# xXCoffeeColaXc/WeatherConverter

Measured on AMD Instinct MI355X. Metric: 256x256 images/sec (T=1000 DDPM sample), higher is better.
Workload: dtype fp32-class (f16x3: 2-piece fp16 split MFMA, fp32 accumulate); 1 GPU; DDPM reverse sampling, UNet config.yaml @ 256px, 16 images/GPU, T=1000, 127 timed steps from t=999; global_batch=16, image_size=256, parallelism=single GPU, devices=1, hip_graph=True, stream_groups=2, x_finite=True

## Files before the change

weatherconverter_amd/csrc/wc_wino.hip:

```cpp
#include <stdlib.h>

#include "wc_x6.hpp"

#ifndef WC_ABL
#define WC_ABL 0
#endif
#ifndef WC_WINO_SCALAR
#define WC_WINO_SCALAR 0
#endif

namespace {

using namespace wcx6;

constexpr int NT = 256;

WC_DEVICE void wino_lds16(__amdgpu_buffer_rsrc_t srd, void* dst, unsigned voff, int soff) {
    __builtin_amdgcn_raw_ptr_buffer_load_lds(srd, (__attribute__((address_space(3))) void*)dst, 16, voff, soff, 0, 0);
}

struct WDev {
    const float* src0;
    int C0, ldc0;
    const float* scale;
    const float* shift;
    const float* src1;
    int C1, ldc1;
    int B, H, W, N;
    const void* w;
    const float* bias;
    const float* temb;
    int temb_ld;
    const float* res;
    int ldres;
    float* out;
    int ldo;
    int nck0, nck1;
    int a_exp;
    const float* abound;
    const float* wsinv;
    float* absmax;
    float* gn_part;
    int gn_ncb, gn_sw, gn_c0, gn_np64;
    int tiles_x, tiles_y, ntiles_n;
    const unsigned char* vpre;
    long vimg;
    const float* gb_x;
    int gb_ldx, gb_silu;
    const float* gb_sc0;
    const float* gb_sh0;
    const float* gb_gamma;
    const float* gb_beta;
    float* gb_part;
    float* gb_part3;
};

WC_DEVICE float wino_silu_grad(float y) {
    const float s = 1.0f / (1.0f + __expf(-y));
    return s * (1.0f + y * (1.0f - s));
}

constexpr int VPL = WC_SINGLE16 ? 8 : 16;

template <int TH, int BN, int MB = 2, int NW = 4, bool VP = false>
struct WTile {
    static constexpr int NT = 64 * NW;
    static constexpr int WAVES_N = BN / 32;
    static constexpr int WAVES_M = NW / WAVES_N;
    static_assert(WAVES_N * WAVES_M == NW && WAVES_M * 4 * MB == TH, "each wave owns 4 MB rows x 8 tiles x 32 channels");
    static constexpr int PBN = BN > 128 ? 128 : BN;
    static constexpr int HR = TH + 2;
    static constexpr int PSTR = HR * 128 + (VP ? 0 : 16);
    static constexpr int DPIECES = VPL * HR * 8 / 64;
    static_assert(!VP || VPL * HR * 8 == DPIECES * 64, "VP: the halo stage is a whole number of 1-KiB pieces");
    static constexpr int DPW = (DPIECES + NW - 1) / NW;
    static constexpr int HSTAGE = 16 * PSTR;
    static constexpr int CPSTR = TH * 128 + 16;
    static constexpr int CSTAGE = 8 * CPSTR;
    static constexpr int ITEMS = HR * 16;
    static constexpr int I_PER_T = (ITEMS + NT - 1) / NT;
    static constexpr int C_PER_T = TH * 16 * 4 / NT;
    static constexpr int BSTEP = PBN * 64;
    static constexpr int STEPS = 12;
};

WC_DEVICE int wg_grp(int r) { return ((r >= 4 && r < 12) || (r >= 16 && r < 20) || r >= 28) ? 1 : 0; }
WC_DEVICE int wg_idx(int r) { return r < 4 ? r : r < 12 ? r - 4 : r < 20 ? r - 8 : r < 28 ? r - 12 : r - 16; }
WC_DEVICE int wg_row(int r) { return 2 * wg_grp(r) + (wg_idx(r) >> 3); }
WC_DEVICE int wg_tile(int r) { return wg_idx(r) & 7; }

template <int TH, int BN, int PRO, bool RES, int MB = 2, int NW = 4>
__global__ __launch_bounds__(64 * NW) __attribute__((amdgpu_waves_per_eu(MB == 4 ? 1 : 2, MB == 4 ? 1 : 2)))
void conv3x3_wino_kernel(WDev p) {
    static_assert((PRO == 2 || PRO == 0 || PRO == 3) && !(PRO == 0 && RES),
                  "GN+SiLU (+ residual), pre-split GN+SiLU (+ residual) or one raw segment");
    constexpr bool VP = PRO == 3;
    using T = WTile<TH, BN, MB, NW, VP>;
    constexpr int NT = T::NT;
    extern __shared__ __attribute__((aligned(16))) unsigned char smem[];
    unsigned char* const cbase = smem + 2 * T::HSTAGE;

    const int tid = threadIdx.x;
    const int lane = tid & 63;
    const int wave = tid >> 6;
    const int wm = wave / T::WAVES_N;
    const int wn = wave % T::WAVES_N;

    const int nblk = gridDim.x;
    int bid = blockIdx.x;
    {
        int q = nblk / 8, r = nblk % 8, xcd = bid % 8;
        bid = (xcd < r ? xcd * (q + 1) : r * (q + 1) + (xcd - r) * q) + bid / 8;
    }
    const int tile_n = bid % p.ntiles_n;
    int tt = bid / p.ntiles_n;
    const int txi = tt % p.tiles_x;
    tt /= p.tiles_x;
    const int tyi = tt % p.tiles_y;
    const int b = tt / p.tiles_y;
    const int y0 = tyi * TH, x0 = txi * 16, n0 = tile_n * BN;

    int s_exp = p.a_exp;
    if ((RES || PRO == 0) && p.abound) {
        const float bnd = p.abound[b];
        const int e = (int)((__float_as_uint(bnd) >> 23) & 0xffu) - 127;
        if (bnd > 0.f) s_exp = min(s_exp, (PRO == 0 ? 12 : 13) - e);
        s_exp = max(s_exp, -100);
    }
    const float ascale = ldexpf(1.0f, s_exp), ainv = ldexpf(1.0f, -s_exp);
    const int S0 = T::STEPS * p.nck0;
    const int S = S0 + (RES ? p.nck1 : 0);
    constexpr bool RI = RES && (T::C_PER_T <= 2 || MB == 4);
    const int nri = RI ? min(p.nck0, p.nck1) : 0;
    const int ntail = RES ? p.nck1 - nri : 0;
    constexpr int WPT = T::PBN / 32;
    const unsigned wtile = (unsigned)(tile_n * (BN / T::PBN) + wn / WPT) * (unsigned)(S * T::BSTEP);

    const __amdgpu_buffer_rsrc_t srd0 = make_srd(p.src0);
    const __amdgpu_buffer_rsrc_t srd1 = make_srd(RES ? p.src1 : p.src0);
    const __amdgpu_buffer_rsrc_t srdw = make_srd(p.w);
    const __amdgpu_buffer_rsrc_t srdsc = make_srd(PRO == 2 ? p.scale : p.src0);
    const __amdgpu_buffer_rsrc_t srdsh = make_srd(PRO == 2 ? p.shift : p.src0);
    const __amdgpu_buffer_rsrc_t srdv = make_srd(VP ? (const void*)(p.vpre + (long)b * p.vimg) : (const void*)p.src0);
    unsigned voff[VP ? T::DPW : 1];
    if constexpr (VP) {
#pragma unroll
        for (int i = 0; i < T::DPW; ++i) {
            const int f = (wave + NW * i) * 64 + lane;
            const int P = f / (T::HR * 8), r = (f >> 3) % T::HR, tl = f & 7;
            const int y = y0 - 1 + r;
            voff[i] = (unsigned)y < (unsigned)p.H ? (unsigned)(((P * p.H + y) * (p.W / 2) + (x0 >> 1) + tl) * 16) : OOB;
        }
    }
    const int vchunk = VPL * p.H * (p.W / 2) * 16;
    auto dma_halo = [&](int c, int hs) {
        if constexpr (VP) {
            unsigned char* dst = smem + hs * T::HSTAGE + wave * 1024;
#pragma unroll
            for (int i = 0; i < T::DPW; ++i)
                if (T::DPIECES % NW == 0 || wave + NW * i < T::DPIECES)
                    wino_lds16(srdv, dst + i * NW * 1024, voff[i], c * vchunk);
        }
    };

    const int q = tid & 3;
    int hbase[T::I_PER_T];
    unsigned hin[T::I_PER_T];
    int hwr[T::I_PER_T];
    const int hpx = p.ldc0 * 4;
#pragma unroll
    for (int j = 0; j < T::I_PER_T; ++j) {
        const int i = tid + NT * j;
        const int hrow = i >> 4, tp = (i >> 2) & 3;
        const bool valid = i < T::ITEMS;
        const int iy = y0 - 1 + hrow;
        hin[j] = 0;
#pragma unroll
        for (int k = 0; k < 6; ++k) {
            const int ix = x0 - 1 + 4 * tp + k;
            const bool inb = valid && (unsigned)iy < (unsigned)p.H && (unsigned)ix < (unsigned)p.W;
            hin[j] |= (inb ? 1u : 0u) << k;
        }
        hbase[j] = (((b * p.H + iy) * p.W + x0 - 1 + 4 * tp) * p.ldc0 + 4 * q) * 4;
        hwr[j] = valid ? (q >> 1) * T::PSTR + (hrow * 8 + 2 * tp) * 16 + (q & 1) * 8 : -1;
    }
    f32x4 rh[T::I_PER_T][6];
    f32x4 rsc, rsh;
    auto load_ss = [&](int c) {
        if constexpr (PRO == 2) {
            const unsigned o = (unsigned)(b * p.C0 + c * 16 + 4 * q) * 4u;
            rsc = bload_f4(srdsc, o);
            rsh = bload_f4(srdsh, o);
        }
    };
    auto load_slot = [&](int j, int c) {
#pragma unroll
        for (int k = 0; k < 6; ++k)
            rh[j][k] = bload_f4s(srd0, ((hin[j] >> k) & 1u) ? (unsigned)(hbase[j] + k * hpx) : OOB, c * 64);
    };
    auto load_halo = [&](int c) {
        if constexpr (VP) return;
#pragma unroll
        for (int j = 0; j < T::I_PER_T; ++j) load_slot(j, c);
        load_ss(c);
    };
#if WC_WINO_SCALAR
    const float cu = -1.4426950408889634f * ainv;
    auto prologue = [&](int j, int k0, int k1) {
        if constexpr (PRO == 2) {
            if (j == 0 && k0 == 0) {
                rsc = rsc * ascale;
                rsh = rsh * ascale;
            }
        }
        auto act = [&](f32x4 a) {
#pragma unroll
            for (int e = 0; e < 4; ++e) {
                float v;
                if constexpr (PRO == 2) {
                    const float ap = __builtin_fmaf(a[e], rsc[e], rsh[e]);
                    const float r = __builtin_amdgcn_rcpf(1.0f + __builtin_amdgcn_exp2f(ap * cu));
                    v = ap * r;
                } else {
                    v = a[e] * ascale;
                }
                a[e] = v;
            }
            return a;
        };
#pragma unroll
        for (int k = k0; k < k1; ++k) {
            const f32x4 zero = {0.f, 0.f, 0.f, 0.f};
#if WC_WINO_SCALAR == 2
            rh[j][k] = ((hin[j] >> k) & 1u) ? act(rh[j][k]) : zero;
#else
            const f32x4 a = act(rh[j][k]);
            rh[j][k] = ((hin[j] >> k) & 1u) ? a : zero;
#endif
        }
    };
#else
    auto prologue = [&](int j, int k0, int k1) {
#pragma unroll
        for (int k = k0; k < k1; ++k) {
            f32x4 a = rh[j][k];
            if constexpr (PRO == 2 && !(WC_ABL & 2)) {
                a = a * rsc + rsh;
                if constexpr (!(WC_ABL & 1)) {
                    a.x = silu_fast(a.x); a.y = silu_fast(a.y);
                    a.z = silu_fast(a.z); a.w = silu_fast(a.w);
                }
            }
            rh[j][k] = ((hin[j] >> k) & 1u) ? a * ascale : f32x4{0.f, 0.f, 0.f, 0.f};
        }
    };
#endif
    auto transform = [&](int j, int t, int hs, int p0 = 0, int p1 = 4) {
        if (hwr[j] < 0) return;
        unsigned char* base = smem + hs * T::HSTAGE + hwr[j] + t * 16;
        const f32x4 d0 = rh[j][2 * t], d1 = rh[j][2 * t + 1], d2 = rh[j][2 * t + 2], d3 = rh[j][2 * t + 3];
#if WC_WINO_SCALAR
        f32x4 V[4];
#pragma unroll
        for (int e = 0; e < 4; ++e) {
            V[0][e] = d0[e] - d2[e];
            V[1][e] = d1[e] + d2[e];
            V[2][e] = d2[e] - d1[e];
            V[3][e] = d1[e] - d3[e];
        }
#else
        const f32x4 V[4] = {d0 - d2, d1 + d2, d2 - d1, d1 - d3};
#endif
#pragma unroll
        for (int pos = p0; pos < p1; ++pos) {
            u32x2 a0, a1;
            split2_f16(V[pos], a0, a1);
            unsigned char* d = base + pos * 2 * T::PSTR;
            *reinterpret_cast<u32x2*>(d) = a0;
            *reinterpret_cast<u32x2*>(d + 8 * T::PSTR) = a1;
        }
    };
    auto write_items = [&](int hs) {
        if constexpr (VP) return;
#pragma unroll
        for (int j = 0; j < T::I_PER_T; ++j) {
            prologue(j, 0, 6);
            transform(j, 0, hs);
            transform(j, 1, hs);
        }
    };

    f32x4 rc[2][RES ? T::C_PER_T : 1];
    const int cpx = (tid >> 2) & 15, crow0 = tid >> 6;
    const unsigned coff0 = (unsigned)(((b * p.H + y0 + crow0) * p.W + x0 + cpx) * p.ldc1 + 4 * q);
    const unsigned cstep = (unsigned)(NW * p.W * p.ldc1);
    const int cwr0 = (cpx & 1) * 2 * T::CPSTR + (q >> 1) * T::CPSTR + (crow0 * 8 + (cpx >> 1)) * 16 + (q & 1) * 8;
    auto load_centre = [&](auto P, int c, bool live = true) {
        constexpr int PV = decltype(P)::value;
        const unsigned v = live ? coff0 * 4u : OOB;
#pragma unroll
        for (int j = 0; j < T::C_PER_T; ++j)
            rc[PV][j] = bload_f4s(srd1, v, (int)(((unsigned)j * cstep + (unsigned)c * 16u) * 4u));
    };
    auto write_centre = [&](auto P, int cs) {
        constexpr int PV = decltype(P)::value;
        unsigned char* base = cbase + cs * T::CSTAGE + cwr0;
        const float sg = (cpx & 1) ? -ascale : ascale;
#pragma unroll
        for (int j = 0; j < T::C_PER_T; ++j) {
            u32x2 a0, a1;
            split2_f16(rc[PV][j] * sg, a0, a1);
            unsigned char* d = base + j * NW * 8 * 16;
            *reinterpret_cast<u32x2*>(d) = a0;
            *reinterpret_cast<u32x2*>(d + 4 * T::CPSTR) = a1;
        }
    };

    const int l32 = lane & 31;
    const int half = lane >> 5;
    int abase[MB];
#pragma unroll
    for (int mb = 0; mb < MB; ++mb) abase[mb] = ((4 * MB * wm + 4 * mb + wg_row(l32)) * 8 + wg_tile(l32)) * 16;
    const unsigned wlane = (unsigned)(half * T::PBN * 16 + ((wn % WPT) * 32 + l32) * 16);

    u32x4 wreg[3][2];
    auto load_w = [&](int set, int st) {
        int s = st < S0 ? st : S0 + nri + (st - S0);
        s = s < S ? s : S - 1;
        const int off = (int)(wtile + (unsigned)s * T::BSTEP);
#pragma unroll
        for (int pc = 0; pc < 2; ++pc) wreg[set][pc] = bload_u4s(srdw, wlane + (unsigned)(pc * 2 * T::PBN * 16), off);
    };
    u32x4 wres[2];
    auto load_wres = [&](int r) {
        const int s = S0 + r < S ? S0 + r : S - 1;
        const int off = (int)(wtile + (unsigned)s * T::BSTEP);
#pragma unroll
        for (int pc = 0; pc < 2; ++pc) wres[pc] = bload_u4s(srdw, wlane + (unsigned)(pc * 2 * T::PBN * 16), off);
    };

    f32x16 acc[4][MB];
#pragma unroll
    for (int i = 0; i < 4; ++i)
#pragma unroll
        for (int j = 0; j < MB; ++j)
#pragma unroll
            for (int r = 0; r < 16; ++r) acc[i][j][r] = 0.f;

    u32x4 fa[2][MB][2];
    auto read_a = [&](int fs, int hs, int dy, int pos) {
        const unsigned char* ha = smem + hs * T::HSTAGE + (pos * 2 + half) * T::PSTR + dy * 128;
#pragma unroll
        for (int mb = 0; mb < MB; ++mb)
#pragma unroll
            for (int pc = 0; pc < 2; ++pc)
                fa[fs][mb][pc] = *reinterpret_cast<const u32x4*>(ha + pc * 8 * T::PSTR + abase[mb]);
    };
    auto mfma_a = [&](int fs, int set, int pos) {
#pragma unroll
        for (int mb = 0; mb < MB; ++mb) acc[pos][mb] = mfma_f16(fa[fs][mb][0], wreg[set][0], acc[pos][mb]);
#pragma unroll
        for (int mb = 0; mb < MB; ++mb) {
            acc[pos][mb] = mfma_f16c(fa[fs][mb][0], wreg[set][1], acc[pos][mb]);
            acc[pos][mb] = mfma_f16c(fa[fs][mb][1], wreg[set][0], acc[pos][mb]);
        }
    };
    auto compute_res = [&](const u32x4 (&w)[2], int cs) {
        const unsigned char* ca = cbase + cs * T::CSTAGE + half * T::CPSTR;
#pragma unroll
        for (int r = 0; r < 2; ++r) {
            u32x4 fr[MB][2];
#pragma unroll
            for (int mb = 0; mb < MB; ++mb)
#pragma unroll
                for (int pc = 0; pc < 2; ++pc)
                    fr[mb][pc] = *reinterpret_cast<const u32x4*>(ca + (pc * 4 + r * 2) * T::CPSTR + abase[mb]);
#pragma unroll
            for (int mb = 0; mb < MB; ++mb) {
                f32x16& a = acc[r ? 3 : 0][mb];
                a = mfma_f16(fr[mb][0], w[0], a);
                a = mfma_f16c(fr[mb][0], w[1], a);
                a = mfma_f16c(fr[mb][1], w[0], a);
            }
        }
    };

    const std::integral_constant<int, 0> I0;
    const std::integral_constant<int, 1> I1;
    const int pv0 = (p.nck0 - 1) & 1;
    load_halo(0);
    dma_halo(0, pv0);
    if constexpr (RI) load_centre(I0, 0, nri > 0);
    load_w(0, 0);
    load_w(1, 1);
    write_items(pv0);
    if constexpr (RI) write_centre(I0, pv0);
    if constexpr (VP) asm volatile("s_waitcnt vmcnt(0)" ::: "memory");
    __syncthreads();
    constexpr int HALO_AT = T::I_PER_T == 1 ? 2 : 3;
    auto load_at = [](int j) { return T::I_PER_T == 1 ? 2 : (j == 0 ? 3 : 7); };
    auto pro_at = [](int j) { return j == 0 ? 5 : 9; };
    auto slot_work = [&](int j, int k, int hs) {
        if constexpr (VP) return;
        if constexpr (WC_ABL & 4) {
            if (k >= 0 && k < 3) prologue(j, 2 * k, 2 * k + 2);
            return;
        }
        if constexpr (T::I_PER_T == 1) {
            if (k >= 0 && k < 3) prologue(j, 2 * k, 2 * k + 2);
            if (k >= 3 && k < 7) transform(j, (k - 3) >> 1, hs, ((k - 3) & 1) * 2, ((k - 3) & 1) * 2 + 2);
        } else {
            if (k == 0) prologue(j, 0, 6);
            if (k == 1 || k == 2) transform(j, k - 1, hs);
        }
    };
    auto chunk = [&](auto P, auto L, int c) {
        constexpr int PV = decltype(P)::value;
        constexpr bool LAST = decltype(L)::value != 0;
        read_a(0, PV, 0, 0);
#pragma unroll
        for (int st = 0; st < T::STEPS; ++st) {
            if (!(WC_ABL & 8) || c == 0) load_w((st + 2) % 3, T::STEPS * c + st + 2);
            if constexpr (!LAST) {
#pragma unroll
                for (int j = 0; j < T::I_PER_T; ++j)
                    if (!(WC_ABL & 32) && st == load_at(j)) load_slot(j, c + 1);
                if (st == HALO_AT) {
                    dma_halo(c + 1, PV ^ 1);
                    load_ss(c + 1);
                    if constexpr (RI) load_centre(I0, c + 1, c + 1 < nri);
                }
            } else if constexpr (RES) {
                if (st == HALO_AT) load_centre(I0, nri, ntail > 0);
                if (st == HALO_AT + 1) load_centre(I1, nri + 1, ntail > 1);
            }
            if constexpr (RI) {
                if (st == 9) load_wres(c);
            }
            __builtin_amdgcn_sched_barrier(0);
            if (st + 1 < T::STEPS && (!(WC_ABL & 64) || c == 0)) read_a((st + 1) & 1, PV, (st + 1) >> 2, (st + 1) & 3);
            mfma_a(st & 1, st % 3, st & 3);
            if constexpr (!LAST) {
#pragma unroll
                for (int j = 0; j < T::I_PER_T; ++j) slot_work(j, st - pro_at(j), PV ^ 1);
                if constexpr (RI) {
                    if (st == 9) write_centre(I0, PV ^ 1);
                }
            }
        }
        if constexpr (RES) {
            if constexpr (RI) {
                if (c < nri) compute_res(wres, PV);
            }
            if constexpr (LAST) {
                if (ntail > 0) write_centre(I0, 1);
            }
        }
        if constexpr (VP && !LAST) asm volatile("s_waitcnt vmcnt(4)" ::: "memory");
        if constexpr (!(WC_ABL & 16)) __syncthreads();
    };
    const std::integral_constant<int, 0> NL;
    const std::integral_constant<int, 1> LL;
    {
        int c = 0;
        if (pv0) chunk(I1, NL, c++);
        for (; c + 1 < p.nck0 - 1; c += 2) {
            chunk(I0, NL, c);
            chunk(I1, NL, c + 1);
        }
        chunk(I0, LL, p.nck0 - 1);
    }
    if constexpr (RES) {
        auto tstep = [&](auto P, int k) {
            constexpr int PV = decltype(P)::value;
            compute_res(wreg[PV], PV ^ 1);
            load_w(PV, S0 + k + 2);
            load_centre(P, nri + k + 2, k + 2 < ntail);
            __builtin_amdgcn_sched_barrier(0);
            if (k + 1 < ntail) write_centre(std::integral_constant<int, PV ^ 1>{}, PV);
            __syncthreads();
        };
        int k = 0;
        for (; k + 1 < ntail; k += 2) {
            tstep(I0, k);
            tstep(I1, k + 1);
        }
        if (k < ntail) tstep(I0, k);
    }

    const long img_px = (long)b * p.H * p.W;
    const __amdgpu_buffer_rsrc_t srd_out = make_srd(p.out + img_px * p.ldo);
    const __amdgpu_buffer_rsrc_t srd_res = make_srd(p.res ? p.res + img_px * p.ldres : p.out);
    const int n = n0 + wn * 32 + l32;
    const bool nok = n < p.N;
    float eadd = (nok && p.bias) ? p.bias[n] : 0.f;
    if (nok && p.temb) eadd += p.temb[b * p.temb_ld + n];
    const float emul = nok ? p.wsinv[n] * ainv : 0.f;
    float vmax = 0.f;
    float gs1 = 0.f, gs2 = 0.f, gs3 = 0.f;
    const int so_px = 4 * p.ldo;
    const int so_rs = 4 * p.ldres;
#pragma unroll
    for (int mb = 0; mb < MB; ++mb) {
        unsigned vo[4], vr[4];
#pragma unroll
        for (int j = 0; j < 4; ++j) {
            const int row = 8 * j + 4 * half;
            const int pix = (y0 + 4 * MB * wm + 4 * mb + wg_row(row)) * p.W + x0 + 2 * wg_tile(row);
            vo[j] = (unsigned)(pix * p.ldo + n) * 4u;
            vr[j] = (unsigned)(pix * p.ldres + (nok ? n : 0)) * 4u;
        }
        float rv[2][16];
        if (p.res) {
#pragma unroll
            for (int r = 0; r < 16; ++r) {
                rv[0][r] = bload_f1s(srd_res, vr[r >> 2], (r & 3) * 2 * so_rs);
                rv[1][r] = bload_f1s(srd_res, vr[r >> 2], ((r & 3) * 2 + 1) * so_rs);
            }
        }
#pragma unroll
        for (int r = 0; r < 16; ++r) {
            const float m0 = acc[0][mb][r], m1 = acc[1][mb][r], m2 = acc[2][mb][r], m3 = acc[3][mb][r];
            float ya = ((m0 + m1) + m2) * emul + eadd;
            float yb = ((m1 - m2) - m3) * emul + eadd;
            if (p.res) {
                ya += rv[0][r];
                yb += rv[1][r];
            }
            acc[0][mb][r] = ya;
            acc[1][mb][r] = yb;
            vmax = fmaxf(vmax, fmaxf(fabsf(ya), fabsf(yb)));
        }
        if constexpr (PRO == 0) {
            if (p.gb_part) {
                const __amdgpu_buffer_rsrc_t srd_x = make_srd(p.gb_x + img_px * p.gb_ldx);
                const int so_x = 4 * p.gb_ldx;
                float xv[2][16];
#pragma unroll
                for (int r = 0; r < 16; ++r) {
                    const int j = r >> 2;
                    const int row = 8 * j + 4 * half;
                    const int pix = (y0 + 4 * MB * wm + 4 * mb + wg_row(row)) * p.W + x0 + 2 * wg_tile(row);
                    const unsigned vx = nok ? (unsigned)(pix * p.gb_ldx + n) * 4u : OOB;
                    xv[0][r] = bload_f1s(srd_x, vx, (r & 3) * 2 * so_x);
                    xv[1][r] = bload_f1s(srd_x, vx, ((r & 3) * 2 + 1) * so_x);
                }
                const long bn = (long)b * p.N + (nok ? n : 0);
                const float sc0 = p.gb_sc0[bn], sh0 = p.gb_sh0[bn];
                const float ga = p.gb_gamma ? p.gb_gamma[nok ? n : 0] : 1.f;
                const float be = p.gb_beta ? p.gb_beta[nok ? n : 0] : 0.f;
#pragma unroll
                for (int r = 0; r < 16; ++r)
#pragma unroll
                    for (int e = 0; e < 2; ++e) {
                        const float xh = xv[e][r] * sc0 + sh0;
                        float d = acc[e][mb][r];
                        if (p.gb_silu) d *= wino_silu_grad(ga * xh + be);
                        gs1 += d;
                        gs2 += d * xh;
                        gs3 += xh;
                    }
            }
        }
        if (nok) {
            if constexpr (WC_ABL & 128) {
                float sum = 0.f;
#pragma unroll
                for (int r = 0; r < 16; ++r) sum += acc[0][mb][r] + acc[1][mb][r];
                if (sum == 1234.5678f) bstore_f1s(srd_out, vo[0], 0, sum);
            } else {
#pragma unroll
                for (int r = 0; r < 16; ++r) {
                    bstore_f1s(srd_out, vo[r >> 2], (r & 3) * 2 * so_px, acc[0][mb][r]);
                    bstore_f1s(srd_out, vo[r >> 2], ((r & 3) * 2 + 1) * so_px, acc[1][mb][r]);
                }
            }
        }
    }
    if (!nok) vmax = 0.f;
    if (p.absmax) block_absmax_atomic(p.absmax, b, vmax);
    if constexpr (PRO == 0) {
        if (p.gb_part) {
            gs1 += __shfl_xor(gs1, 32, 64);
            gs2 += __shfl_xor(gs2, 32, 64);
            gs3 += __shfl_xor(gs3, 32, 64);
            const int splits = p.tiles_y * p.tiles_x * T::WAVES_M;
            const long sp = (long)b * splits + ((long)tyi * p.tiles_x + txi) * T::WAVES_M + wm;
            if (nok && half == 0) {
                p.gb_part[(sp * p.N + n) * 2] = gs1;
                p.gb_part[(sp * p.N + n) * 2 + 1] = gs2;
                if (p.gb_part3) p.gb_part3[sp * p.N + n] = gs3;
            }
        }
    }
    if (p.gn_part) {
        const int r4 = tyi * (TH / 4) + MB * wm;
#pragma unroll
        for (int mb = 0; mb < MB; ++mb) {
            const f32x16 blk[2][1] = {{acc[0][mb]}, {acc[1][mb]}};
            GnTile g{p.gn_part, p.gn_ncb, p.gn_sw,
                     (long)b * p.gn_np64 + (long)(((r4 + mb) >> 1) * p.tiles_x + txi) * 2 + ((r4 + mb) & 1),
                     (p.gn_c0 + n0 + wn * 32) / 32};
            gn_tile_partials(blk, g, p.N - n0 - wn * 32 >= 32 ? 1 : 0);
        }
    }
}

template <int TH, int BN, int PRO, bool RES, int MB = 2, int NW = 4>
int launch_wino(const WDev& d, hipStream_t stream) {
    using T = WTile<TH, BN, MB, NW, PRO == 3>;
    constexpr int lds = 2 * T::HSTAGE + (RES ? 2 * T::CSTAGE : 0);
    static bool attr_set = false;
    if (!attr_set) {
        hipError_t e = hipFuncSetAttribute(reinterpret_cast<const void*>(&conv3x3_wino_kernel<TH, BN, PRO, RES, MB, NW>),
                                           hipFuncAttributeMaxDynamicSharedMemorySize, lds);
        if (e != hipSuccess) return (int)e;
        attr_set = true;
    }
    WDev p = d;
    p.tiles_x = p.W / 16;
    p.tiles_y = p.H / TH;
    p.ntiles_n = (p.N + BN - 1) / BN;
    dim3 grid(p.B * p.tiles_y * p.tiles_x * p.ntiles_n);
    WC_SET_NAME("conv3x3_wino_kernel", {WC_TI(TH), WC_TI(BN), WC_TI(PRO), WC_TB(RES), WC_TI(MB), WC_TI(NW)});
    hipLaunchKernelGGL((conv3x3_wino_kernel<TH, BN, PRO, RES, MB, NW>), grid, dim3(T::NT), lds, stream, p);
    WC_CHECK_LAUNCH();
    return WC_OK;
}

}

extern "C" int wc_conv3x3_wino_tile_n(int N) { return N <= 64 ? 64 : 128; }

namespace {

int wino_setup(const wc_conv_args* a, const void* w, int64_t w_bytes, int a_exp, const float* w_inv_scale,
               const float* a_bound, WDev& d, int& pro, bool& res, int& BN) {
    if (!a || !w || !a->out || !w_inv_scale) return WC_E_ARG;
    if (a->nseg < 1 || a->nseg > 2) return WC_E_ARG;
    const wc_conv_seg& s0 = a->seg[0];
    if (!s0.src || (s0.scale == nullptr) != (s0.shift == nullptr)) return WC_E_ARG;
    pro = s0.scale ? 2 : 0;
    if (pro == 2 && !s0.silu) return WC_E_ARG;
    if (pro == 0 && (!a_bound || a->nseg != 1)) return WC_E_ARG;
    if (a->act != WC_ACT_NONE) return WC_E_ARG;
    if (a_exp < -60 || a_exp > 60) return WC_E_ARG;
    BN = wc_conv3x3_wino_tile_n(a->N);
    const int TH = BN == 64 ? 16 : 8;
    if (s0.ntaps != 9 || s0.sy != 1 || s0.sx != 1 || s0.kbase != 0) return WC_E_SHAPE;
    for (int t = 0; t < 9; ++t)
        if (s0.dy[t] != t / 3 - 1 || s0.dx[t] != t % 3 - 1) return WC_E_SHAPE;
    if (s0.C <= 0 || s0.C % 16 || s0.ldc % 4 || (reinterpret_cast<uintptr_t>(s0.src) & 15)) return WC_E_SHAPE;
    if (a->B <= 0 || a->N <= 0 || s0.H != a->Hm || s0.W != a->Wm || a->Hm % TH || a->Wm % 16) return WC_E_SHAPE;
    if ((long)a->B * s0.H * s0.W * s0.ldc * 4 >= (1L << 31)) return WC_E_SHAPE;
    if (reinterpret_cast<uintptr_t>(w) & 15) return WC_E_SHAPE;
    d = WDev{};
    d.src0 = s0.src; d.C0 = s0.C; d.ldc0 = s0.ldc; d.scale = s0.scale; d.shift = s0.shift;
    d.nck0 = s0.C / 16;
    res = a->nseg == 2;
    if (res) {
        const wc_conv_seg& s1 = a->seg[1];
        if (!s1.src || s1.scale || !a_bound) return WC_E_ARG;
        if (s1.ntaps != 1 || s1.dy[0] != 0 || s1.dx[0] != 0 || s1.sy != 1 || s1.sx != 1) return WC_E_SHAPE;
        if (s1.H != s0.H || s1.W != s0.W || s1.kbase != 9 * s0.C) return WC_E_SHAPE;
        if (s1.C <= 0 || s1.C % 16 || s1.ldc % 4 || (reinterpret_cast<uintptr_t>(s1.src) & 15)) return WC_E_SHAPE;
        if ((long)a->B * s1.H * s1.W * s1.ldc * 4 >= (1L << 31)) return WC_E_SHAPE;
        d.src1 = s1.src; d.C1 = s1.C; d.ldc1 = s1.ldc; d.nck1 = s1.C / 16;
    }
    if (a->out_nchw || a->Ho != a->Hm || a->Wo != a->Wm || a->osy != 1 || a->osx != 1 || a->ooy || a->oox)
        return WC_E_SHAPE;
    if ((long)a->Hm * a->Wm * a->ldo * 4 >= (1L << 31) || (a->res && (long)a->Hm * a->Wm * a->ldres * 4 >= (1L << 31)))
        return WC_E_SHAPE;
    d.B = a->B; d.H = a->Hm; d.W = a->Wm; d.N = a->N;
    d.w = w; d.bias = a->bias; d.temb = a->temb; d.temb_ld = a->temb_ld;
    d.res = a->res; d.ldres = a->ldres; d.out = a->out; d.ldo = a->ldo;
    d.a_exp = a_exp - 1;
    d.abound = (res || pro == 0) ? a_bound : nullptr;
    d.wsinv = w_inv_scale;
    d.absmax = a->absmax_out;
    d.gn_part = a->gn_part;
    if (a->gn_part) {
        const int sw = a->gn_sw;
        if ((sw != 4 && sw != 8 && sw != 16 && sw != 32) || a->N % 32 || a->gn_c0 % 32 || a->gn_c0 < 0 ||
            a->gn_c0 + a->N > a->gn_ncb * 32 || a->gn_p64 != 0 || a->gn_np64 * 64 != a->Hm * a->Wm)
            return WC_E_SHAPE;
        d.gn_ncb = a->gn_ncb; d.gn_sw = sw; d.gn_c0 = a->gn_c0; d.gn_np64 = a->gn_np64;
    }
    const long ntn = (a->N + BN - 1) / BN;
    if (w_bytes != ntn * (12L * d.nck0 + d.nck1) * BN * 64 || w_bytes >= (1L << 31)) return WC_E_SHAPE;
    return WC_OK;
}

long wino_vimg(int C, int H, int W) { return (long)(C / 16) * VPL * H * (W / 2) * 16; }

#ifndef VS_IPT
#define VS_IPT 4
#endif
template <int NCK>
__global__ __launch_bounds__(256) void wino_vsplit_kernel(const float* __restrict__ src, int ldc, int B, int H,
                                                          int W, int C, const float* __restrict__ scale,
                                                          const float* __restrict__ shift, int a_exp1,
                                                          const float* __restrict__ res_bound,
                                                          unsigned char* __restrict__ vout, long vimg) {
    extern __shared__ __attribute__((aligned(16))) f32x4 act[];
    const int R = 256 / W, ngrp = C / (16 * NCK), nyb = (H + R - 1) / R;
    const int kg = blockIdx.x % ngrp;
    const int yb = (blockIdx.x / ngrp) % nyb;
    const int b = blockIdx.x / (ngrp * nyb);
    const int y0 = yb * R;
    const int tid = threadIdx.x;
    int s_exp = a_exp1;
    if (res_bound) {
        const float bnd = res_bound[b];
        const int e = (int)((__float_as_uint(bnd) >> 23) & 0xffu) - 127;
        if (bnd > 0.f) s_exp = min(s_exp, 13 - e);
        s_exp = max(s_exp, -100);
    }
    const float ascale = ldexpf(1.0f, s_exp);
    const int W2 = W + 2, items = R * W2 * 4 * NCK, cstride = R * W2 * 5;
    const int qt = tid % (4 * NCK), ct = kg * 16 * NCK + 4 * qt;
    const f32x4 sct = *reinterpret_cast<const f32x4*>(scale + (long)b * C + ct);
    const f32x4 sht = *reinterpret_cast<const f32x4*>(shift + (long)b * C + ct);
    for (int i0 = tid; i0 < items; i0 += VS_IPT * 256) {
        f32x4 v[VS_IPT];
        bool inb[VS_IPT];
        int slot[VS_IPT];
#pragma unroll
        for (int u = 0; u < VS_IPT; ++u) {
            const int i = min(i0 + u * 256, items - 1);
            const int px = (i / (4 * NCK)) % W2 - 1, r = (i / (4 * NCK)) / W2;
            const int y = y0 + r;
            inb[u] = (unsigned)px < (unsigned)W && y < H;
            v[u] = *reinterpret_cast<const f32x4*>(src + ((long)(b * H + min(y, H - 1)) * W + min(max(px, 0), W - 1)) * ldc + ct);
            slot[u] = (qt >> 2) * cstride + (r * W2 + px + 1) * 5 + (qt & 3);
        }
#pragma unroll
        for (int u = 0; u < VS_IPT; ++u) {
            if (i0 + u * 256 >= items) break;
            f32x4 a = v[u] * sct + sht;
            a.x = silu_fast(a.x); a.y = silu_fast(a.y);
            a.z = silu_fast(a.z); a.w = silu_fast(a.w);
            act[slot[u]] = inb[u] ? a * ascale : f32x4{0.f, 0.f, 0.f, 0.f};
        }
    }
    __syncthreads();
    const int T2 = W / 2;
    const int t = tid % T2, h = (tid / T2) & 1, r = tid / W;
    const int y = y0 + r;
    if (r >= R || y >= H) return;
    const long plane = (long)H * T2 * 16;
    const long frag = ((long)y * T2 + t) * 16;
#pragma unroll
    for (int ck = 0; ck < NCK; ++ck) {
        unsigned char* vb = vout + (long)b * vimg + (long)(kg * NCK + ck) * VPL * H * T2 * 16;
        u32x2 pc[2][4][2];
#pragma unroll
        for (int qq = 0; qq < 2; ++qq) {
            const f32x4* ar = act + ck * cstride + (r * W2 + 2 * t) * 5 + 2 * h + qq;
            const f32x4 d0 = ar[0], d1 = ar[5], d2 = ar[10], d3 = ar[15];
            const f32x4 V[4] = {d0 - d2, d1 + d2, d2 - d1, d1 - d3};
#pragma unroll
            for (int pos = 0; pos < 4; ++pos) split2_f16(V[pos], pc[qq][pos][0], pc[qq][pos][1]);
        }
#pragma unroll
        for (int pos = 0; pos < 4; ++pos)
#pragma unroll
            for (int piece = 0; piece < VPL / 8; ++piece)
                *reinterpret_cast<u32x4*>(vb + (piece * 8 + pos * 2 + h) * plane + frag) =
                    u32x4{pc[0][pos][piece].x, pc[0][pos][piece].y, pc[1][pos][piece].x, pc[1][pos][piece].y};
    }
}

}

extern "C" int wc_conv3x3_wino_f16x3(const wc_conv_args* a, const void* w, int64_t w_bytes, int a_exp,
                                     const float* w_inv_scale, const float* a_bound, void* stream) {
    WDev d;
    int pro, BN;
    bool res;
    const int st = wino_setup(a, w, w_bytes, a_exp, w_inv_scale, a_bound, d, pro, res, BN);
    if (st != WC_OK) return st;
    hipStream_t s = reinterpret_cast<hipStream_t>(stream);
    if (pro == 0) return BN == 64 ? launch_wino<16, 64, 0, false>(d, s) : launch_wino<8, 128, 0, false>(d, s);
    if (BN == 64) return res ? launch_wino<16, 64, 2, true>(d, s) : launch_wino<16, 64, 2, false>(d, s);
    return res ? launch_wino<8, 128, 2, true>(d, s) : launch_wino<8, 128, 2, false>(d, s);
}

extern "C" int wc_conv3x3_wino_gnb_splits(int N, int H, int W) {
    const int BN = wc_conv3x3_wino_tile_n(N), TH = BN == 64 ? 16 : 8;
    if (N <= 0 || H <= 0 || W <= 0 || H % TH || W % 16) return -1;
    const int waves_m = 4 / (BN / 32);
    return (H / TH) * (W / 16) * waves_m;
}

extern "C" int wc_conv3x3_wino_f16x3_gnb(const wc_conv_args* a, const void* w, int64_t w_bytes, int a_exp,
                                         const float* w_inv_scale, const float* a_bound, const wc_gnb_epi* g,
                                         void* stream) {
    WDev d;
    int pro, BN;
    bool res;
    const int st = wino_setup(a, w, w_bytes, a_exp, w_inv_scale, a_bound, d, pro, res, BN);
    if (st != WC_OK) return st;
    if (pro != 0 || !g || !g->x || !g->sc0 || !g->sh0 || !g->part) return WC_E_ARG;
    if (g->ldx < d.N || g->splits != wc_conv3x3_wino_gnb_splits(d.N, d.H, d.W)) return WC_E_SHAPE;
    if ((long)d.B * d.H * d.W * g->ldx * 4 >= (1L << 31)) return WC_E_SHAPE;
    d.gb_x = g->x; d.gb_ldx = g->ldx; d.gb_silu = g->silu ? 1 : 0;
    d.gb_sc0 = g->sc0; d.gb_sh0 = g->sh0; d.gb_gamma = g->gamma; d.gb_beta = g->beta;
    d.gb_part = g->part; d.gb_part3 = g->part3;
    hipStream_t s = reinterpret_cast<hipStream_t>(stream);
    return BN == 64 ? launch_wino<16, 64, 0, false>(d, s) : launch_wino<8, 128, 0, false>(d, s);
}

extern "C" int wc_wino_vsplit_bytes(int B, int C, int H, int W, int64_t* bytes) {
    if (!bytes || B <= 0 || C <= 0 || C % 16 || H <= 0 || W <= 0 || W % 16) return WC_E_SHAPE;
    *bytes = (int64_t)B * wino_vimg(C, H, W);
    return WC_OK;
}

extern "C" int wc_wino_vsplit_f16x3(const wc_conv_args* a, int a_exp, const float* a_bound, void* vout, int64_t v_bytes,
                                    void* stream) {
    if (!a || !vout || a->nseg < 1 || a->nseg > 2) return WC_E_ARG;
    const wc_conv_seg& s0 = a->seg[0];
    if (!s0.src || !s0.scale || !s0.shift || !s0.silu) return WC_E_ARG;
    if (a->nseg == 2 && !a_bound) return WC_E_ARG;
    if (a_exp < -60 || a_exp > 60) return WC_E_ARG;
    if (s0.C <= 0 || s0.C % 16 || s0.ldc % 4 || (reinterpret_cast<uintptr_t>(s0.src) & 15) || s0.W % 16)
        return WC_E_SHAPE;
    if ((reinterpret_cast<uintptr_t>(vout) & 15) || v_bytes != (int64_t)a->B * wino_vimg(s0.C, s0.H, s0.W))
        return WC_E_SHAPE;
    if (s0.W > 256) return WC_E_SHAPE;
    const int R = 256 / s0.W;
    const int nck = s0.C % 32 == 0 ? 2 : 1;
    const long nblk = (long)a->B * ((s0.H + R - 1) / R) * (s0.C / (16 * nck));
    const size_t lds = (size_t)nck * R * (s0.W + 2) * 5 * sizeof(f32x4);
    if (lds > 64 * 1024) return WC_E_SHAPE;
    hipStream_t st = reinterpret_cast<hipStream_t>(stream);
    const float* rb = a->nseg == 2 ? a_bound : nullptr;
    unsigned char* vo = reinterpret_cast<unsigned char*>(vout);
    const long vimg = wino_vimg(s0.C, s0.H, s0.W);
    if (nck == 2) {
        WC_SET_NAME("wino_vsplit_kernel", {WC_TI(2)});
        hipLaunchKernelGGL(wino_vsplit_kernel<2>, dim3((unsigned)nblk), dim3(256), lds, st, s0.src, s0.ldc, a->B, s0.H,
                           s0.W, s0.C, s0.scale, s0.shift, a_exp - 1, rb, vo, vimg);
    } else {
        WC_SET_NAME("wino_vsplit_kernel", {WC_TI(1)});
        hipLaunchKernelGGL(wino_vsplit_kernel<1>, dim3((unsigned)nblk), dim3(256), lds, st, s0.src, s0.ldc, a->B, s0.H,
                           s0.W, s0.C, s0.scale, s0.shift, a_exp - 1, rb, vo, vimg);
    }
    WC_CHECK_LAUNCH();
    return WC_OK;
}

extern "C" int wc_conv3x3_wino_f16x3_vp(const wc_conv_args* a, const void* w, int64_t w_bytes, int a_exp,
                                        const float* w_inv_scale, const float* a_bound, const void* vpre,
                                        int64_t v_bytes, void* stream) {
    WDev d;
    int pro, BN;
    bool res;
    const int st = wino_setup(a, w, w_bytes, a_exp, w_inv_scale, a_bound, d, pro, res, BN);
    if (st != WC_OK) return st;
    if (pro != 2 || !vpre || (reinterpret_cast<uintptr_t>(vpre) & 15)) return WC_E_ARG;
    d.vimg = wino_vimg(d.C0, d.H, d.W);
    if (v_bytes != (int64_t)d.B * d.vimg || d.vimg >= (1L << 31)) return WC_E_SHAPE;
    d.vpre = reinterpret_cast<const unsigned char*>(vpre);
    hipStream_t s = reinterpret_cast<hipStream_t>(stream);
    if (BN == 64) return res ? launch_wino<16, 64, 3, true>(d, s) : launch_wino<16, 64, 3, false>(d, s);
    return res ? launch_wino<8, 128, 3, true>(d, s) : launch_wino<8, 128, 3, false>(d, s);
}

extern "C" int wc_conv3x3_wino_f16x3_vp8(const wc_conv_args* a, const void* w, int64_t w_bytes, int a_exp,
                                         const float* w_inv_scale, const float* a_bound, const void* vpre,
                                         int64_t v_bytes, void* stream) {
    WDev d;
    int pro, BN;
    bool res;
    const int st = wino_setup(a, w, w_bytes, a_exp, w_inv_scale, a_bound, d, pro, res, BN);
    if (st != WC_OK) return st;
    if (pro != 2 || !vpre || (reinterpret_cast<uintptr_t>(vpre) & 15)) return WC_E_ARG;
    if (BN != 128 || d.N % 256) return WC_E_SHAPE;
    d.vimg = wino_vimg(d.C0, d.H, d.W);
    if (v_bytes != (int64_t)d.B * d.vimg || d.vimg >= (1L << 31)) return WC_E_SHAPE;
    d.vpre = reinterpret_cast<const unsigned char*>(vpre);
    hipStream_t s = reinterpret_cast<hipStream_t>(stream);
    return res ? launch_wino<8, 256, 3, true, 2, 8>(d, s) : launch_wino<8, 256, 3, false, 2, 8>(d, s);
}

namespace {

__device__ double wino_u(const float* row, int C0, int ky, int pos, int c) {
    const double g0 = row[(ky * 3 + 0) * C0 + c], g1 = row[(ky * 3 + 1) * C0 + c], g2 = row[(ky * 3 + 2) * C0 + c];
    switch (pos) {
        case 0: return g0;
        case 1: return ((g0 + g1) + g2) * 0.5;
        case 2: return ((g0 - g1) + g2) * 0.5;
        default: return g2;
    }
}

__device__ void wino_u8(const float* row, int ld, int ky, int pos, int c, double* v) {
    f32x4 g[3][2];
#pragma unroll
    for (int k = 0; k < 3; ++k) {
        g[k][0] = *reinterpret_cast<const f32x4*>(row + (ky * 3 + k) * ld + c);
        g[k][1] = *reinterpret_cast<const f32x4*>(row + (ky * 3 + k) * ld + c + 4);
    }
#pragma unroll
    for (int e = 0; e < 8; ++e) {
        const double g0 = g[0][e >> 2][e & 3], g1 = g[1][e >> 2][e & 3], g2 = g[2][e >> 2][e & 3];
        v[e] = pos == 0 ? g0 : pos == 1 ? ((g0 + g1) + g2) * 0.5 : pos == 2 ? ((g0 - g1) + g2) * 0.5 : g2;
    }
}

__device__ void pack_wino_row(const float* row3, int ld, bool vec, const float* rres, bool live, int n, int C0, int C1,
                              int BN, short* __restrict__ out, float* __restrict__ wsinv) {
    const int c8 = C0 / 8, n0 = 12 * c8, nall = n0 + C1 / 8;
    auto values = [&](int it, double* v) {
        if (it < n0) {
            const int kp = it / c8, c = (it - kp * c8) * 8;
            if (vec) {
                wino_u8(row3, ld, kp / 4, kp % 4, c, v);
            } else {
#pragma unroll
                for (int e = 0; e < 8; ++e) v[e] = wino_u(row3, ld, kp / 4, kp % 4, c + e);
            }
        } else {
            const int c = (it - n0) * 8;
#pragma unroll
            for (int e = 0; e < 8; ++e) v[e] = rres[c + e];
        }
    };
    double m = 0.0;
    if (live) {
        for (int it = threadIdx.x; it < nall; it += blockDim.x) {
            double v[8];
            values(it, v);
#pragma unroll
            for (int e = 0; e < 8; ++e) m = fmax(m, fabs(v[e]));
        }
    }
    __shared__ double red[256];
    red[threadIdx.x] = m;
    __syncthreads();
    for (int s = 128; s > 0; s >>= 1) {
        if ((int)threadIdx.x < s) red[threadIdx.x] = fmax(red[threadIdx.x], red[threadIdx.x + s]);
        __syncthreads();
    }
    const double amax = red[0];
    int sw = 0;
    if (amax > 0.0) {
        int e;
        const double mant = frexp(amax, &e);
        sw = (mant == 0.5 ? 15 : 14) - e;
        sw = sw < -60 ? -60 : sw > 60 ? 60 : sw;
    }
    const double scale = ldexp(1.0, sw);
    if (threadIdx.x == 0) wsinv[n] = ldexpf(1.0f, -sw);
    const int T = n / BN, nn = n % BN;
    const long rowlen = (long)(12 * (C0 / 16) + C1 / 16) * 2 * 2 * BN * 8;
    short* trow = out + (long)T * rowlen;
    const int plane = 2 * BN * 8;
    for (int it = threadIdx.x; it < nall; it += blockDim.x) {
        double v[8];
        if (live) values(it, v);
        else
#pragma unroll
            for (int e = 0; e < 8; ++e) v[e] = 0.0;
        long o;
        if (it < n0) {
            const int kp = it / c8, c = (it - kp * c8) * 8, ky = kp / 4, pos = kp % 4;
            const int chunk = c / 16, kh = (c % 16) / 8;
            o = ((((long)(chunk * 3 + ky) * 4 + pos) * 2 * 2 + kh) * BN + nn) * 8;
        } else {
            const int c = (it - n0) * 8;
            const int chunk = c / 16, kh = (c % 16) / 8;
            o = (long)(C0 / 16) * 12 * 2 * 2 * BN * 8 + (((long)chunk * 2 * 2 + kh) * BN + nn) * 8;
        }
        unsigned hp[4], lp[4];
#pragma unroll
        for (int e = 0; e < 8; e += 2) {
            unsigned short h0, l0, h1, l1;
            float a = (float)(v[e] * scale), b = (float)(v[e + 1] * scale);
            asm volatile("" : "+v"(a), "+v"(b));
            split2_one(a, h0, l0);
            split2_one(b, h1, l1);
            hp[e / 2] = (unsigned)h0 | ((unsigned)h1 << 16);
            lp[e / 2] = (unsigned)l0 | ((unsigned)l1 << 16);
        }
        *reinterpret_cast<u32x4*>(trow + o) = u32x4{hp[0], hp[1], hp[2], hp[3]};
        *reinterpret_cast<u32x4*>(trow + o + plane) = u32x4{lp[0], lp[1], lp[2], lp[3]};
    }
}

__global__ __launch_bounds__(256) void pack_wino_kernel(const float* __restrict__ w, int K, int N, int C0, int C1,
                                                        int BN, short* __restrict__ out, float* __restrict__ wsinv) {
    const int n = blockIdx.x;
    const bool live = n < N;
    const float* row = w + (long)(live ? n : 0) * K;
    pack_wino_row(row, C0, false, row + 9 * C0, live, n, C0, C1, BN, out, wsinv);
}

__device__ void stage_row3(const float* __restrict__ w, bool transposed, int N, int n, int C0, float* row3) {
    const int lim = 9 * C0, ld = C0 + 4;
    for (int i0 = threadIdx.x; i0 < lim; i0 += 8 * 256) {
        float v[8];
#pragma unroll
        for (int k = 0; k < 8; ++k) {
            const int i = i0 + k * 256;
            const int c = i / 9, t = i - 9 * c;
            v[k] = i < lim ? (transposed ? w[((long)c * N + n) * 9 + t] : w[(long)n * lim + i]) : 0.f;
        }
#pragma unroll
        for (int k = 0; k < 8; ++k) {
            const int i = i0 + k * 256;
            const int c = i / 9, t = i - 9 * c;
            if (i < lim) row3[(transposed ? 8 - t : t) * ld + c] = v[k];
        }
    }
}

template <bool TRANSPOSED>
__global__ __launch_bounds__(256) void pack_wino_raw_kernel(const float* __restrict__ w, const float* __restrict__ wres,
                                                            int N, int C0, int C1, int BN, short* __restrict__ out,
                                                            float* __restrict__ wsinv) {
    extern __shared__ float row3[];
    const int n = blockIdx.x;
    const bool live = n < N;
    if (live) stage_row3(w, TRANSPOSED, N, n, C0, row3);
    __syncthreads();
    pack_wino_row(row3, C0 + 4, true, wres + (long)(live ? n : 0) * C1, live, n, C0, C1, BN, out, wsinv);
}

__global__ __launch_bounds__(256) void pack_wino_batch_kernel(const wc_wino_pack_job* __restrict__ jobs, int njobs) {
    extern __shared__ float row3[];
    __shared__ int s_wg0[256];
    const int g = blockIdx.x;
    const bool lds = njobs <= 256;
    if (lds && (int)threadIdx.x < njobs) s_wg0[threadIdx.x] = jobs[threadIdx.x].wg0;
    __syncthreads();
    int lo = 0, hi = njobs - 1;
    while (lo < hi) {
        const int mid = (lo + hi + 1) >> 1;
        if ((lds ? s_wg0[mid] : jobs[mid].wg0) <= g) lo = mid;
        else hi = mid - 1;
    }
    const wc_wino_pack_job jb = jobs[lo];
    const int n = g - jb.wg0;
    const bool live = n < jb.N;
    const int C0 = jb.C0, N = jb.N;
    if (live) stage_row3(jb.w, jb.transposed != 0, N, n, C0, row3);
    __syncthreads();
    pack_wino_row(row3, C0 + 4, true, jb.wres + (long)(live ? n : 0) * jb.C1, live, n, C0, jb.C1, jb.BN,
                  reinterpret_cast<short*>(jb.out), jb.wsinv);
}

}

extern "C" int wc_pack_wino(const float* w, int N, int C0, int C1, void* out, int64_t out_bytes, float* w_inv_scale,
                            void* stream) {
    if (!w || !out || !w_inv_scale) return WC_E_ARG;
    if (N <= 0 || C0 <= 0 || C0 % 16 || C1 < 0 || C1 % 16) return WC_E_SHAPE;
    const int BN = wc_conv3x3_wino_tile_n(N);
    const long ntn = (N + BN - 1) / BN;
    if (out_bytes != ntn * (12L * (C0 / 16) + C1 / 16) * BN * 64) return WC_E_SHAPE;
    hipLaunchKernelGGL(pack_wino_kernel, dim3((unsigned)(ntn * BN)), dim3(256), 0, reinterpret_cast<hipStream_t>(stream),
                       w, 9 * C0 + C1, N, C0, C1, BN, reinterpret_cast<short*>(out), w_inv_scale);
    wc_last_kernel = "pack_wino_kernel";
    WC_CHECK_LAUNCH();
    return WC_OK;
}

extern "C" int wc_pack_wino_batch(const wc_wino_pack_job* jobs, int njobs, int total_wg, int max_c0, void* stream) {
    if (!jobs || njobs < 0 || total_wg < 0) return WC_E_ARG;
    if (njobs == 0) return WC_OK;
    if (max_c0 <= 0 || 9L * (max_c0 + 4) * 4 > 64 * 1024 || total_wg <= 0) return WC_E_SHAPE;
    hipLaunchKernelGGL(pack_wino_batch_kernel, dim3((unsigned)total_wg), dim3(256), (size_t)9 * (max_c0 + 4) * sizeof(float),
                       reinterpret_cast<hipStream_t>(stream), jobs, njobs);
    wc_last_kernel = "pack_wino_batch_kernel";
    WC_CHECK_LAUNCH();
    return WC_OK;
}

extern "C" int wc_pack_wino_raw(const float* w, const float* wres, int N, int C0, int C1, int transposed, void* out,
                                int64_t out_bytes, float* w_inv_scale, void* stream) {
    if (!w || !out || !w_inv_scale || (C1 && !wres) || (transposed && C1)) return WC_E_ARG;
    if (N <= 0 || C0 <= 0 || C0 % 16 || C1 < 0 || C1 % 16 || 9L * (C0 + 4) * 4 > 64 * 1024) return WC_E_SHAPE;
    const int BN = wc_conv3x3_wino_tile_n(N);
    const long ntn = (N + BN - 1) / BN;
    if (out_bytes != ntn * (12L * (C0 / 16) + C1 / 16) * BN * 64) return WC_E_SHAPE;
    const size_t lds = (size_t)9 * (C0 + 4) * sizeof(float);
    hipStream_t s = reinterpret_cast<hipStream_t>(stream);
    if (transposed)
        hipLaunchKernelGGL(pack_wino_raw_kernel<true>, dim3((unsigned)(ntn * BN)), dim3(256), lds, s, w, wres, N, C0, C1,
                           BN, reinterpret_cast<short*>(out), w_inv_scale);
    else
        hipLaunchKernelGGL(pack_wino_raw_kernel<false>, dim3((unsigned)(ntn * BN)), dim3(256), lds, s, w, wres, N, C0,
                           C1, BN, reinterpret_cast<short*>(out), w_inv_scale);
    wc_last_kernel = "pack_wino_raw_kernel";
    WC_CHECK_LAUNCH();
    return WC_OK;
}
```

Baseline: 0.6834 images/s.

## Load Winograd halo with 4 pixels per lane and share overlap via ds_bpermute

```diff
diff --git a/weatherconverter_amd/csrc/wc_wino.hip b/weatherconverter_amd/csrc/wc_wino.hip
--- a/weatherconverter_amd/csrc/wc_wino.hip
+++ b/weatherconverter_amd/csrc/wc_wino.hip
@@ -77,8 +77,8 @@
     static constexpr int HSTAGE = 16 * PSTR;
     static constexpr int CPSTR = TH * 128 + 16;
     static constexpr int CSTAGE = 8 * CPSTR;
-    static constexpr int ITEMS = HR * 16;
-    static constexpr int I_PER_T = (ITEMS + NT - 1) / NT;
+    static constexpr int IROWS = 3;
+    static constexpr int I_PER_T = (HR + IROWS * NW - 1) / (IROWS * NW);
     static constexpr int C_PER_T = TH * 16 * 4 / NT;
     static constexpr int BSTEP = PBN * 64;
     static constexpr int STEPS = 12;
@@ -164,26 +164,33 @@
     };
 
     const int q = tid & 3;
+    const int irow = lane / 20, iseg = (lane % 20) >> 2;
+    auto slot_rows = [](int j) { return T::HR - T::IROWS * NW * j < T::IROWS * NW ? T::HR - T::IROWS * NW * j : T::IROWS * NW; };
+    auto slot_live = [&](int j) {
+        if (slot_rows(j) >= NW) return true;
+        return __builtin_amdgcn_readfirstlane(wave) < slot_rows(j);
+    };
     int hbase[T::I_PER_T];
     unsigned hin[T::I_PER_T];
     int hwr[T::I_PER_T];
     const int hpx = p.ldc0 * 4;
 #pragma unroll
     for (int j = 0; j < T::I_PER_T; ++j) {
-        const int i = tid + NT * j;
-        const int hrow = i >> 4, tp = (i >> 2) & 3;
-        const bool valid = i < T::ITEMS;
+        const int per = slot_rows(j) / NW, extra = slot_rows(j) % NW;
+        const int hrow = T::IROWS * NW * j + wave * per + min(wave, extra) + irow;
+        const bool valid = irow < per + (wave < extra ? 1 : 0);
         const int iy = y0 - 1 + hrow;
         hin[j] = 0;
 #pragma unroll
-        for (int k = 0; k < 6; ++k) {
-            const int ix = x0 - 1 + 4 * tp + k;
-            const bool inb = valid && (unsigned)iy < (unsigned)p.H && (unsigned)ix < (unsigned)p.W;
+        for (int k = 0; k < 4; ++k) {
+            const int ix = x0 - 1 + 4 * iseg + k;
+            const bool inb = valid && (iseg < 4 || k < 2) && (unsigned)iy < (unsigned)p.H && (unsigned)ix < (unsigned)p.W;
             hin[j] |= (inb ? 1u : 0u) << k;
         }
-        hbase[j] = (((b * p.H + iy) * p.W + x0 - 1 + 4 * tp) * p.ldc0 + 4 * q) * 4;
-        hwr[j] = valid ? (q >> 1) * T::PSTR + (hrow * 8 + 2 * tp) * 16 + (q & 1) * 8 : -1;
-    }
+        hbase[j] = (((b * p.H + iy) * p.W + x0 - 1 + 4 * iseg) * p.ldc0 + 4 * q) * 4;
+        hwr[j] = valid && iseg < 4 ? (q >> 1) * T::PSTR + (hrow * 8 + 2 * iseg) * 16 + (q & 1) * 8 : -1;
+    }
+    const int xlane = ((lane + 4) & 63) << 2;
     f32x4 rh[T::I_PER_T][6];
     f32x4 rsc, rsh;
     auto load_ss = [&](int c) {
@@ -195,7 +202,7 @@
     };
     auto load_slot = [&](int j, int c) {
 #pragma unroll
-        for (int k = 0; k < 6; ++k)
+        for (int k = 0; k < 4; ++k)
             rh[j][k] = bload_f4s(srd0, ((hin[j] >> k) & 1u) ? (unsigned)(hbase[j] + k * hpx) : OOB, c * 64);
     };
     auto load_halo = [&](int c) {
@@ -255,6 +262,15 @@
         }
     };
 #endif
+    auto exchange = [&](int j) {
+#pragma unroll
+        for (int k = 0; k < 2; ++k)
+#pragma unroll
+            for (int e = 0; e < 4; ++e) {
+                const float v = rh[j][k][e];
+                rh[j][4 + k][e] = __int_as_float(__builtin_amdgcn_ds_bpermute(xlane, __float_as_int(v)));
+            }
+    };
     auto transform = [&](int j, int t, int hs, int p0 = 0, int p1 = 4) {
         if (hwr[j] < 0) return;
         unsigned char* base = smem + hs * T::HSTAGE + hwr[j] + t * 16;
@@ -284,7 +300,9 @@
         if constexpr (VP) return;
 #pragma unroll
         for (int j = 0; j < T::I_PER_T; ++j) {
-            prologue(j, 0, 6);
+            if (!slot_live(j)) continue;
+            prologue(j, 0, 4);
+            exchange(j);
             transform(j, 0, hs);
             transform(j, 1, hs);
         }
@@ -402,15 +420,18 @@
     auto pro_at = [](int j) { return j == 0 ? 5 : 9; };
     auto slot_work = [&](int j, int k, int hs) {
         if constexpr (VP) return;
+        if (k < 0 || k > (T::I_PER_T == 1 ? 6 : 2) || !slot_live(j)) return;
         if constexpr (WC_ABL & 4) {
-            if (k >= 0 && k < 3) prologue(j, 2 * k, 2 * k + 2);
+            if (k < 2) prologue(j, 2 * k, 2 * k + 2);
             return;
         }
         if constexpr (T::I_PER_T == 1) {
-            if (k >= 0 && k < 3) prologue(j, 2 * k, 2 * k + 2);
-            if (k >= 3 && k < 7) transform(j, (k - 3) >> 1, hs, ((k - 3) & 1) * 2, ((k - 3) & 1) * 2 + 2);
+            if (k < 2) prologue(j, 2 * k, 2 * k + 2);
+            if (k == 2) exchange(j);
+            if (k >= 3) transform(j, (k - 3) >> 1, hs, ((k - 3) & 1) * 2, ((k - 3) & 1) * 2 + 2);
         } else {
-            if (k == 0) prologue(j, 0, 6);
+            if (k == 0) prologue(j, 0, 4);
+            if (k == 1) exchange(j);
             if (k == 1 || k == 2) transform(j, k - 1, hs);
         }
     };
```

After: 0.6879 images/s (median of 6 runs). Within noise of the previous version (+0.7%).
